# cvg/diffmvs

Hardware: AMD Instinct MI355X
Metric: depth-maps/sec (640x512, 5 src views) (higher is better)
Workload: dtype f32

## Files before the change

### diffmvs_amd/_lib.py

```python
from __future__ import annotations

import ctypes as C
import os

PKG = os.path.dirname(os.path.abspath(__file__))
HIP_LIB_PATH = os.environ.get("DMVS_LIB") or os.path.join(PKG, "libdmvs_hip.so")

ACT_NONE, ACT_RELU, ACT_SIGMOID, ACT_TANH, ACT_SILU = range(5)
IN_PLAIN, IN_UPSAMPLE2, IN_UNSHUFFLE2, IN_ZEROINSERT2 = range(4)
LAYOUT_NCHW, LAYOUT_NHWC, LAYOUT_NHWC_BF16, LAYOUT_NHWC_F16 = 0, 1, 2, 3
DTYPE_F32, DTYPE_BF16, DTYPE_F16, DTYPE_F32_PLAIN = 0, 1, 2, 3
ARITH_F32, ARITH_BF16, ARITH_SPLIT = 0, 1, 2
EW_DEPTH_TO_DISP, EW_DISP_TO_DEPTH = 0, 1

_P = C.c_void_p
_I = C.c_int32
_F = C.c_float


class Conv2dDesc(C.Structure):
    _fields_ = [
        ("in0", _P), ("in1", _P), ("mul0", _P), ("weight", _P), ("scale", _P), ("shift", _P),
        ("residual", _P), ("gru_z", _P), ("gru_h", _P), ("out", _P), ("gn_stats", _P), ("out_mul", _P),
        ("B", _I), ("c0", _I), ("c1", _I), ("Hin", _I), ("Win", _I), ("Hout", _I), ("Wout", _I),
        ("cout", _I), ("cout_pad", _I), ("kh", _I), ("kw", _I), ("stride", _I), ("pad_h", _I), ("pad_w", _I),
        ("in_mode", _I), ("act", _I), ("res_mode", _I), ("res_after_act", _I),
        ("out_layout", _I), ("out_cstride", _I), ("out_coffset", _I), ("gn_groups", _I), ("post_scale", _F),
        ("gate_cstride", _I), ("arith", _I), ("tune", _I), ("out_mul_c0", _I), ("in0_cstride", _I), ("weight_split", _P),
    ]


class Conv3dDesc(C.Structure):
    _fields_ = [
        ("in_", _P), ("weight", _P), ("scale", _P), ("shift", _P), ("residual", _P), ("out", _P),
        ("B", _I), ("cin", _I), ("cout", _I), ("cout_pad", _I),
        ("Din", _I), ("Hin", _I), ("Win", _I), ("Dout", _I), ("Hout", _I), ("Wout", _I),
        ("stride", _I), ("transposed", _I), ("act", _I), ("tune", _I),
    ]


class GetCostDesc(C.Structure):
    _fields_ = [
        ("ref", _P), ("src", _P), ("rt", _P), ("inv_depth", _P), ("confidence", _P), ("view_w", _P),
        ("disp_min", _P), ("disp_max", _P), ("out_cost", _P), ("out_samples", _P), ("worklist", _P),
        ("B", _I), ("S", _I), ("C", _I), ("G", _I), ("n", _I), ("H", _I), ("W", _I), ("vw_shift", _I),
        ("cost_cstride", _I), ("cost_coffset", _I), ("samp_cstride", _I), ("samp_coffset", _I),
        ("interval", _F), ("min_radius", _F), ("max_radius", _F), ("feat_dtype", _I), ("tune", _I),
    ]


SIGNATURES = {
    "dmvs_abi_version": [],
    "dmvs_conv2d_f32": [C.POINTER(Conv2dDesc), _P],
    "dmvs_featurenet_stem_f32": [_P, _P, _P, _P, _P, _P, _P, _P, _I, _I, _I, _I, _P],
    "dmvs_conv2d_wgrad_workspace_f32": [C.POINTER(Conv2dDesc), C.POINTER(C.c_int64)],
    "dmvs_conv2d_wgrad_f32": [C.POINTER(Conv2dDesc), _P, _P, _P, _P, C.c_int64, _P],
    "dmvs_conv3d_f32": [C.POINTER(Conv3dDesc), _P],
    "dmvs_conv3d_wgrad_workspace_f32": [C.POINTER(Conv3dDesc), C.POINTER(C.c_int64)],
    "dmvs_conv3d_wgrad_f32": [C.POINTER(Conv3dDesc), _P, _P, _P, _P, C.c_int64, _P],
    "dmvs_compose_proj_f32": [_P, _P, _I, _I, _P],
    "dmvs_warp_volume_f32": [_P, _P, _P, _P, _I, _I, _I, _I, _I, _I, _I, _P],
    "dmvs_getcost_quad_f32": [C.POINTER(GetCostDesc), _P],
    "dmvs_warp_corr_init_quad_f32": [_P, _P, _P, _P, _P, _P, _I, _I, _I, _I, _I, _I, _I, _I, _I, _I, _I, _P],
    "dmvs_warp_corr_init_bwd_f32": [_P, _P, _P, _P, _P, _P, _P, _P, _I, _I, _I, _I, _I, _I, _I, _I, _I, _I, _P],
    "dmvs_getcost_bwd_f32": [C.POINTER(GetCostDesc), _P, _P, _P, _P],
    "dmvs_view_aggregate_bwd_f32": [_P, _P, _P, _P, _P, _P, _I, _I, _I, _I, _P],
    "dmvs_view_aggregate_f32": [_P, _P, _P, _I, _I, _I, _I, _P],
    "dmvs_sigmoid_max_d_f32": [_P, _P, _I, _I, _I, _P],
    "dmvs_depth_regress_f32": [_P, _P, _P, _P, _P, _P, _I, _I, _I, _P],
    "dmvs_convex_upsample_f32": [_P, _P, _P, _P, _P, _P, _I, _I, _I, _I, _P],
    "dmvs_mask_upsample4_f32": [_P, _P, _P, _F, _P, _P, _P, _P, _P, _I, _I, _I, _I, _I, _P],
    "dmvs_groupnorm_silu_f32": [_P, _P, _P, _P, _P, _P, _P, _I, _I, _I, _I, _F, _P],
    "dmvs_groupnorm_apply_f32": [_P, _P, _P, _P, _P, _P, _P, _I, _I, _I, _I, _F, _P],
    "dmvs_delta_update_f32": [_P, _P, _P, _F, _P, _P, _P, _I, _I, _I, _I, _P],
    "dmvs_depth_convert_f32": [_P, _P, _P, _P, _I, _I, _I, _P],
    "dmvs_act_slice_f32": [_P, _P, _I, _I, _I, _I, _I, _I, _I, _I, _P],
    "dmvs_upsample_nearest_f32": [_P, _P, _I, _I, _I, _I, _P],
    "dmvs_nchw_to_nhwc_f32": [_P, _P, _I, _I, _I, _P],
    "dmvs_groupnorm_silu_bwd_workspace_f32": [_I, _I, _I, C.POINTER(C.c_int64)],
    "dmvs_groupnorm_silu_bwd_f32": [_P, _P, _P, _P, _P, _P, _P, _P, _P, _P, _P, C.c_int64, _I, _I, _I, _I, _F, _P],
    "dmvs_batchnorm_workspace_f32": [_I, _I, _I, _I, C.POINTER(C.c_int64)],
    "dmvs_batchnorm_train_fwd_f32": [_P, _P, _P, _P, _P, _P, _P, _P, _P, C.c_int64, _I, _I, _I, _I, _I, _F, _F, _I, _P],
    "dmvs_batchnorm_train_bwd_f32": [_P, _P, _P, _P, _P, _P, _P, _P, _P, _P, C.c_int64, _I, _I, _I, _I, _I, _I, _P],
    "dmvs_geo_consistency_f32": [_P, _P, _P, _P, _P, _I, _I, _F, _F, _P, _P, _I, _I, _I, _I, _I, _P],
    "dmvs_sumsq_f32": [_P, C.c_int64, _P, _P],
    "dmvs_adamw_step_f32": [_P, _P, _P, _P, C.c_int64, _F, _F, _F, _F, _F, _I, _F, _P, _F, _P],
    "dmvs_view_select_scores_f64": [_P, _P, _P, _P, _P, C.c_int64, C.c_int64, _P, _I, C.c_double, C.c_double, C.c_double, _P, _P, _P],
    "dmvs_cloud_nn_dist_f32": [_P, C.c_int64, _P, C.c_int64, _P, _P, C.c_int64, _P, C.c_double, _P, _F, _P, _P, _P],
    "dmvs_cloud_stats_f32": [_P, _P, C.c_int64, _F, _P, _I, C.c_double, _I, _P, _P],
    "dmvs_cloud_nn_index_f32": [_P, C.c_int64, _P, C.c_int64, _P, _P, C.c_int64, _P, C.c_double, _P, _F, _P, _P, _P, _P, _P],
    "dmvs_cloud_pair_moments_f64": [_P, C.c_int64, _P, _P, C.c_int64, _P, _P, _F, _P, _P, C.c_double, C.c_double, C.c_double, _I, _P, _P],
    "dmvs_cloud_crop_prism_f32": [_P, C.c_int64, _P, _P, _I, _I, C.c_double, C.c_double, _P, _P],
    "dmvs_depth_stats_f32": [_P, _P, _P, C.c_int64, C.c_int64, _P, _I, C.c_double, C.c_double, C.c_double, C.c_double, _I, _P, _P],
    "dmvs_cloud_splat_zmin_f32": [_P, C.c_int64, _P, _P, C.c_int64, _I, _I, C.c_double, C.c_double, C.c_double, _I, _I, _P, _P, _P, _P],
    "dmvs_cloud_splat_sum_f32": [_P, C.c_int64, _P, _P, C.c_int64, _I, _I, C.c_double, C.c_double, C.c_double, C.c_double, C.c_double, _I, _P, _P, _P, _P],
    "dmvs_depth_normals_f32": [_P, _P, _P, C.c_int64, _I, _I, _I, C.c_double, _I, _P, _P, _P],
}
VIEW_SELECT_MAX_IMAGES, VIEW_SELECT_MAX_LIST = 16384, 1 << 23
CLOUD_MAX_RINGS, CLOUD_MAX_KEY_BITS, CLOUD_MAX_THRESHOLDS = 1024, 62, 16
CLOUD_MOMENTS, CLOUD_MAX_POLYGON = 20, 256
DEPTH_MAX_THRESHOLDS, DEPTH_SLOTS = 8, 7
SPLAT_VIEW_CHUNK, SPLAT_VIEW_DOUBLES, SPLAT_SLOTS, SPLAT_MAX_RADIUS, SPLAT_NO_PRETEST = 8, 15, 4, 16, 0x1
NORMAL_MAX_RADIUS, NORMAL_CAM_DOUBLES, NORMAL_VIEW_CHUNK, NORMAL_SLOTS = 4, 27, 8, 4
ABI_VERSION = 4
TUNE_NO_WALK, TUNE_PIECES4, TUNE_NO_LEAN, TUNE_1X1_TILED, TUNE_NO_TALL, TUNE_TALL = 0x4, 0x8, 0x100, 0x200, 0x400, 0x800
TUNE3D_PIECES4, TUNE3D_S2_DIRECT, TUNE3D_NO_PAIR = 0x1, 0x2, 0x4
TUNE_SWEEP_GLOBAL = 0x1
TUNE_WGRAD_ACCUMULATE = 0x1000
TUNE_SPLIT_ALL = 0x20000
TUNE_STEM_EXACT = 0x40000


def tune_xcd_group(n: int) -> int:
    return (int(n) & 7) << 14


def tune3d_xcd_group(n: int) -> int:
    return (int(n) & 7) << 4
TUNE_BWD_INTERLEAVED, BWD_GATHER_INTERLEAVED = 0x1, 2


def tune_tile_wx(n: int) -> int:
    return n & 3


def tune_tile_mt(n: int) -> int:
    return (n & 7) << 4


class DmvsError(RuntimeError):
    pass


class Lib:

    def __init__(self, path: str):
        if not os.path.exists(path):
# ... 27 lines not shown
```

### diffmvs_amd/build.py

```python
from __future__ import annotations

import os
import subprocess
import sys

PKG = os.path.dirname(os.path.abspath(__file__))
ROOT = os.path.dirname(PKG)
CSRC = os.path.join(PKG, "csrc")
LIB = os.path.join(PKG, "libdmvs_hip.so")
PROBE_LIB = os.path.join(PKG, "libdmvs_probe.so")
PROBE_SOURCES = ["probe/getcost_probe.hip", "probe/random_line_gather.hip"]
SOURCES = ["conv2d_k33.hip", "conv2d_k55.hip", "conv2d_k77.hip", "conv2d_k15.hip", "conv2d.hip", "stem.hip", "conv3d.hip", "warp_quad.hip", "warp_bwd.hip", "warp_bwd_win.hip", "warp_init_bwd_win.hip", "misc.hip", "mask_upsample.hip", "optim.hip", "norm.hip", "fusion.hip", "view_select.hip", "cloud_eval.hip", "cloud_register.hip", "depth_eval.hip", "cloud_render.hip", "depth_normals.hip"]


def _deps():
    out = [os.path.join(ROOT, "include", "dmvs.h"), os.path.join(ROOT, "include", "dmvs_probe.h")]
    for base, _, files in os.walk(CSRC):
        out += [os.path.join(base, f) for f in files]
    return out


def _stale() -> bool:
    if not os.path.exists(LIB) or not os.path.exists(PROBE_LIB):
        return True
    t = min(os.path.getmtime(LIB), os.path.getmtime(PROBE_LIB))
    return any(os.path.getmtime(d) > t for d in _deps())


def build_hip(force: bool = False, save_temps: bool = False, verbose: bool = True) -> str:
    if not force and not _stale():
        return LIB
    import time
    t_start = time.time()
    hipcc = os.environ.get("HIPCC", "/opt/rocm/bin/hipcc")
    flags = ["--offload-arch=gfx950", "-O3", "-std=c++17", "-fPIC",
             "-I", os.path.join(ROOT, "include"), "-I", CSRC,
             "-munsafe-fp-atomics",
             "-Wall", "-Wno-unused-function"]
    objdir = os.path.join(ROOT, "build", "temps" if save_temps else "obj")
    os.makedirs(objdir, exist_ok=True)
    if save_temps:
        flags += ["-save-temps=obj", "-Rpass-analysis=kernel-resource-usage"]

    hdr_t = max(os.path.getmtime(d) for d in _deps() if d.endswith(".h"))

    def compile_one(src):
        obj = os.path.join(objdir, src.replace("/", "_") + ".o")
        if not force and not save_temps and os.path.exists(obj) and os.path.getmtime(obj) > max(hdr_t, os.path.getmtime(os.path.join(CSRC, src))):
            return obj
        cmd = [hipcc] + flags + ["-c", os.path.join(CSRC, src), "-o", obj]
        if verbose:
            print("[diffmvs_amd.build]", " ".join(cmd), flush=True)
        t0 = time.time()
        subprocess.run(cmd, check=True, cwd=objdir if save_temps else ROOT)
        os.utime(obj, (t0, t0))
        return obj

    from concurrent.futures import ThreadPoolExecutor
    with ThreadPoolExecutor(max_workers=min(len(SOURCES), os.cpu_count() or 4)) as pool:
        objs = list(pool.map(compile_one, SOURCES + PROBE_SOURCES))
    for lib, lobjs in ((LIB, objs[:len(SOURCES)]), (PROBE_LIB, objs[len(SOURCES):])):
        link = [hipcc, "--offload-arch=gfx950", "-shared", "-fPIC"] + lobjs + ["-o", lib]
        if verbose:
            print("[diffmvs_amd.build]", " ".join(link), flush=True)
        subprocess.run(link, check=True, cwd=ROOT)
        os.utime(lib, (t_start, t_start))
    return LIB


if __name__ == "__main__":
    build_hip(force="--force" in sys.argv, save_temps="--save-temps" in sys.argv)
    print(LIB)
```

### diffmvs_amd/engine.py

```python
from __future__ import annotations

import math
import os
from typing import Callable, Dict, List, Optional

import torch
import torch.nn.functional as F

from . import ops as K
from .ops import Ops, PackedConv, pack_conv2d, pack_conv3d

_RATIOS = [4, 2, 1]
_MULTS = [(1,), (1, 2), (1, 2, 4)]


def _bn(sd, p):
    return {k: sd[f"{p}.{k}"] for k in ("weight", "bias", "running_mean", "running_var")}


def _cw(sd, p, **kw):
    return pack_conv2d(sd[p + ".conv.weight"], sd.get(p + ".conv.bias"),
                       bn=_bn(sd, p + ".bn") if (p + ".bn.weight") in sd else None, **kw)


def pack_feature(sd, p="feature", g4=False, feat_dtype=torch.float32):
    order = (lambda w: w[K.g4_channels(w.shape[0], feat_dtype).to(w.device)].contiguous()) if g4 else (lambda w: w)
    f = {"conv0.0": _cw(sd, p + ".conv0.0", pad=1), "conv0.1": _cw(sd, p + ".conv0.1", pad=1)}
    for i in (1, 2, 3):
        f[f"conv{i}.0"] = _cw(sd, f"{p}.conv{i}.0", stride=2, pad=2)
        f[f"conv{i}.1"], f[f"conv{i}.2"] = _cw(sd, f"{p}.conv{i}.1", pad=1), _cw(sd, f"{p}.conv{i}.2", pad=1)
    f["out1"] = pack_conv2d(order(sd[p + ".out1.weight"]))
    f["inner1"] = pack_conv2d(sd[p + ".inner1.weight"], sd[p + ".inner1.bias"])
    f["out2"] = pack_conv2d(order(sd[p + ".out2.weight"]), pad=1)
    if (p + ".out3.weight") in sd:
        f["inner2"] = pack_conv2d(sd[p + ".inner2.weight"], sd[p + ".inner2.bias"])
        f["out3"] = pack_conv2d(order(sd[p + ".out3.weight"]), pad=1)
    return f


def run_feature(o: Ops, f, x, layout=K.LAYOUT_NHWC, feat_dtype=torch.float32):
    R = K.ACT_RELU
    c0 = o.featurenet_stem(f["conv0.0"], f["conv0.1"], x)
    c1 = o.conv2d(f["conv1.0"], c0, act=R)
    c1 = o.conv2d(f["conv1.2"], o.conv2d(f["conv1.1"], c1, act=R), act=R)
    c2 = o.conv2d(f["conv2.2"], o.conv2d(f["conv2.1"], o.conv2d(f["conv2.0"], c1, act=R), act=R), act=R)
    c3 = o.conv2d(f["conv3.2"], o.conv2d(f["conv3.1"], o.conv2d(f["conv3.0"], c2, act=R), act=R), act=R)
    out = {"stage1": o.conv2d(f["out1"], c3, out_layout=layout, out_dtype=feat_dtype)}
    intra = o.conv2d(f["inner1"], c2, residual=c3, res_mode=K.IN_UPSAMPLE2)
    out["stage2"] = o.conv2d(f["out2"], intra, out_layout=layout, out_dtype=feat_dtype)
    if "out3" in f:
        intra = o.conv2d(f["inner2"], c1, residual=intra, res_mode=K.IN_UPSAMPLE2)
        out["stage3"] = o.conv2d(f["out3"], intra, out_layout=layout, out_dtype=feat_dtype)
    return out


def pack_context_trunk(sd, p="context"):
    c = {"conv1": _cw(sd, p + ".conv1", pad=1)}
    for li in (1, 2, 3):
        for bi in (0, 1):
            q = f"{p}.layer{li}.{bi}"
            c[f"{li}.{bi}.conv1"] = _cw(sd, q + ".conv1", stride=(2 if bi == 0 else 1), pad=1)
            c[f"{li}.{bi}.conv2"] = _cw(sd, q + ".conv2", pad=1)
            if bi == 0:
                c[f"{li}.{bi}.down"] = _cw(sd, q + ".downsample", stride=2, pad=1)
    return c


def run_context_trunk(o: Ops, c, x):
    R = K.ACT_RELU
    x = o.conv2d(c["conv1"], x, act=R)
    taps = {}
    for li in (1, 2, 3):
        y = o.conv2d(c[f"{li}.0.conv1"], x, act=R)
        xd = o.conv2d(c[f"{li}.0.down"], x)
        x = o.conv2d(c[f"{li}.0.conv2"], y, residual=xd, act=R)
        y = o.conv2d(c[f"{li}.1.conv1"], x, act=R)
        x = o.conv2d(c[f"{li}.1.conv2"], y, residual=x, act=R)
        taps[3 - li] = x
    return taps


def pack_pvw(sd, p):
    return (pack_conv3d(sd[p + ".conv.0.conv.weight"], bn=_bn(sd, p + ".conv.0.bn")),
            pack_conv3d(sd[p + ".conv.1.weight"], sd[p + ".conv.1.bias"]))


def run_pvw(o: Ops, pk, cor):
    N, _, D, H, W = cor.shape
    x = o.conv3d(pk[1], o.conv3d(pk[0], cor, act=K.ACT_RELU))
    return o.sigmoid_max_d(x.view(N, D, H, W))


def pack_costreg(sd, p):
    reg = {}
    for i, st in ((0, 1), (1, 1), (2, 2), (3, 1), (4, 2), (5, 1)):
        reg[i] = pack_conv3d(sd[f"{p}.conv{i}.conv.weight"], bn=_bn(sd, f"{p}.conv{i}.bn"), stride=st)
    for i in (6, 7):
        reg[i] = pack_conv3d(sd[f"{p}.conv{i}.conv.weight"], bn=_bn(sd, f"{p}.conv{i}.bn"), stride=2, transposed=True)
    reg["prob"] = pack_conv3d(sd[p + ".prob.weight"])
    return reg


def run_costreg(o: Ops, reg, x):
    R = K.ACT_RELU
    c1 = o.conv3d(reg[1], o.conv3d(reg[0], x, act=R), act=R)
    c3 = o.conv3d(reg[3], o.conv3d(reg[2], c1, act=R), act=R)
    x = o.conv3d(reg[5], o.conv3d(reg[4], c3, act=R), act=R)
    x = o.conv3d(reg[6], x, act=R, residual=c3)
    x = o.conv3d(reg[7], x, act=R, residual=c1)
    return o.conv3d(reg["prob"], x)


def pack_mask(sd, p):
    return (pack_conv2d(sd[p + ".0.weight"], sd[p + ".0.bias"], pad=1), pack_conv2d(sd[p + ".2.weight"], sd[p + ".2.bias"]))


def run_mask(o: Ops, pk, context, post_scale=0.25):
    return o.conv2d(pk[1], o.conv2d(pk[0], context, act=K.ACT_RELU), post_scale=post_scale)


def mask_head_fuses(pk, up_ratio) -> bool:
    return up_ratio == 4 and pk[1].cin == 64 and pk[1].cout == 144 and pk[1].scale is None and os.environ.get("DMVS_MASK_FUSE", "1") != "0"


def pack_gru(sd, p):
    g = {}
# ... 440 lines not shown
```

### diffmvs_amd/ops.py

```python
from __future__ import annotations

import ctypes as C
import os
from dataclasses import dataclass
from typing import Optional

import torch

from . import _lib
from ._lib import (ACT_NONE, ACT_RELU, ACT_SIGMOID, ACT_SILU, ACT_TANH, ARITH_BF16, ARITH_F32, ARITH_SPLIT, DTYPE_BF16, DTYPE_F16, DTYPE_F32, IN_PLAIN,
                   IN_UNSHUFFLE2, IN_UPSAMPLE2, IN_ZEROINSERT2, LAYOUT_NCHW, LAYOUT_NHWC, LAYOUT_NHWC_BF16, LAYOUT_NHWC_F16)

CONV_ARITH = {"fp32": ARITH_F32, "bf16": ARITH_BF16, "split": ARITH_SPLIT}
FEATURE_DTYPES = {"fp32": torch.float32, "bf16": torch.bfloat16, "fp16": torch.float16}
_DTYPE_CODE = {torch.float32: DTYPE_F32, torch.bfloat16: DTYPE_BF16, torch.float16: DTYPE_F16}
_NHWC_LAYOUT = {torch.float32: LAYOUT_NHWC, torch.bfloat16: LAYOUT_NHWC_BF16, torch.float16: LAYOUT_NHWC_F16}


def _round_up(x: int, m: int) -> int:
    return (x + m - 1) // m * m


@dataclass
class PackedConv:
# ... 222 lines not shown
            if (x0.dtype != torch.float32 or x0.device != self.device or x0.stride(1) != x0.shape[2] * x0.shape[3] or
                    x0.stride(0) != in0_cstride * x0.shape[2] * x0.shape[3] or x0.stride(3) != 1 or in_mode != IN_PLAIN):
                raise _lib.DmvsError("in0_cstride: x0 must be a channel slice of a contiguous [B,in0_cstride,H,W] tensor, plain input mode")
        self._chk(out_mul)
        if gate_cstride:
            self._chk(*(() if in0_cstride else (x0,)), x1, residual, gru_h)
            for t in (mul0, gru_z):
                if t is not None and (t.dtype != torch.float32 or t.device != self.device or t.stride(1) != t.shape[2] * t.shape[3] or
                                      t.stride(0) != gate_cstride * t.shape[2] * t.shape[3] or t.stride(3) != 1):
                    raise _lib.DmvsError("gate_cstride: mul0 / gru_z must be channel slices of a contiguous [B,gate_cstride,H,W] tensor")
        else:
            self._chk(*(() if in0_cstride else (x0,)), x1, mul0, residual, gru_z, gru_h)
        if out_dtype != torch.float32:
            if out_layout != LAYOUT_NHWC or out is not None:
                raise _lib.DmvsError("16-bit outputs are channel-last feature tensors allocated by conv2d")
            out_layout = _NHWC_LAYOUT[out_dtype]
        else:
            self._chk(out)
        if gn_stats is not None and (gn_stats.dtype != torch.float64 or gn_stats.numel() < x0.shape[0] * gn_groups * 2):
            raise _lib.DmvsError("gn_stats must be float64 with B*groups*2 elements")
        B = x0.shape[0]
        if in_mode == IN_PLAIN:
            c0, Hin, Win = x0.shape[1], x0.shape[2], x0.shape[3]
        elif in_mode in (IN_UPSAMPLE2, IN_ZEROINSERT2):
            c0, Hin, Win = x0.shape[1], x0.shape[2] * 2, x0.shape[3] * 2
        else:
            c0, Hin, Win = x0.shape[1] * 4, x0.shape[2] // 2, x0.shape[3] // 2
        c1 = 0 if x1 is None else x1.shape[1]
        assert c0 + c1 == pc.cin, (c0, c1, pc.cin)
        kh, kw = pc.k
        Hout = (Hin + 2 * pc.pad[0] - kh) // pc.stride + 1
        Wout = (Win + 2 * pc.pad[1] - kw) // pc.stride + 1
        if out_cstride is None:
            out_cstride = pc.cout
        if out is None:
            shape = (B, out_cstride, Hout, Wout) if out_layout == LAYOUT_NCHW else (B, Hout, Wout, out_cstride)
            out = self.empty(*shape, dtype=out_dtype)
        arith = self.conv_arith if arith is None else arith
        wsplit = split_weights(pc) if (arith == ARITH_SPLIT and kh * kw > 1 and out_layout in (LAYOUT_NCHW, LAYOUT_NHWC)) else None
        d = _lib.Conv2dDesc(
            weight_split=_ptr(wsplit),
            in0=_ptr(x0), in1=_ptr(x1), mul0=_ptr(mul0), weight=_ptr(pc.weight), scale=_ptr(pc.scale),
            shift=_ptr(pc.shift), residual=_ptr(residual), gru_z=_ptr(gru_z), gru_h=_ptr(gru_h), out=_ptr(out),
            gn_stats=_ptr(gn_stats), gn_groups=(gn_groups if gn_stats is not None else 0), B=B, c0=c0, c1=c1, Hin=Hin, Win=Win, Hout=Hout, Wout=Wout, cout=pc.cout, cout_pad=pc.cout_pad,
            kh=kh, kw=kw, stride=pc.stride, pad_h=pc.pad[0], pad_w=pc.pad[1], in_mode=in_mode, act=act,
            res_mode=res_mode, res_after_act=int(res_after_act), out_layout=out_layout, out_cstride=out_cstride,
            out_coffset=out_coffset, post_scale=post_scale, gate_cstride=gate_cstride,
            arith=arith, tune=(self.tune["conv2d"] if tune is None else tune),
            out_mul=_ptr(out_mul), out_mul_c0=out_mul_c0, in0_cstride=in0_cstride)
        self._call("dmvs_conv2d_f32", C.byref(d), self.stream())
        if self.timers is not None and "dmvs_conv2d_f32" in self.timers:
            self.timers.setdefault("_conv2d_flops", []).append(2.0 * B * Hout * Wout * pc.cout * pc.cin * kh * kw)
            self.timers.setdefault("_conv2d_shape", []).append((B, pc.cin, pc.cout, kh, kw, pc.stride, Hout, Wout, in_mode, int(mul0 is not None)))
            nb = sum(t.numel() * t.element_size() for t in (x0, x1, mul0, residual, gru_z, gru_h, out_mul) if t is not None)
            self.timers.setdefault("_conv2d_bytes", []).append(nb + B * Hout * Wout * pc.cout * out.element_size())
        return out

    def featurenet_stem(self, pc0: PackedConv, pc1: PackedConv, x, tune=None):
        if isinstance(x, (list, tuple)):
            self._chk(*x)
            Bv, cin, H, W = x[0].shape
            y = self.empty(len(x) * Bv, 8, H, W)
            for v, xv in enumerate(x):
                self._stem_launch(pc0, pc1, xv, y[v * Bv:(v + 1) * Bv], tune)
            return y
        self._chk(x)
        N, cin, H, W = x.shape
        y = self.empty(N, 8, H, W)
        self._stem_launch(pc0, pc1, x, y, tune)
        return y

    def _stem_launch(self, pc0: PackedConv, pc1: PackedConv, x, y, tune=None):
        N, cin, H, W = x.shape
        if not (cin == 3 and pc0.cin == 3 and pc0.cout == 8 and pc1.cin == 8 and pc1.cout == 8 and pc0.k == (3, 3) and
                pc1.k == (3, 3) and pc0.stride == 1 and pc1.stride == 1 and pc0.pad == (1, 1) and pc1.pad == (1, 1) and
                pc0.cout_pad == 8 and pc1.cout_pad == 8):
            raise _lib.DmvsError("featurenet_stem: expects the 3->8->8 3x3 stem of FeatureNet")
        tune = self.tune["stem"] if tune is None else tune
        if self.conv_arith != ARITH_SPLIT:
            tune |= _lib.TUNE_STEM_EXACT
        self._call("dmvs_featurenet_stem_f32", _ptr(x), _ptr(pc0.weight), _ptr(pc0.scale), _ptr(pc0.shift), _ptr(pc1.weight),
                   _ptr(pc1.scale), _ptr(pc1.shift), _ptr(y), N, H, W, tune, self.stream())

    def conv2d_wgrad(self, pc: PackedConv, x0, grad_out, x1=None, *, mul0=None, in_mode=IN_PLAIN, want_bias=False, tune=None,
                     into_gw=None, into_gb=None):
        self._chk(x0, x1, mul0, grad_out, into_gw, into_gb)
        B = x0.shape[0]
        if in_mode == IN_PLAIN:
            c0, Hin, Win = x0.shape[1], x0.shape[2], x0.shape[3]
        elif in_mode in (IN_UPSAMPLE2, IN_ZEROINSERT2):
            c0, Hin, Win = x0.shape[1], x0.shape[2] * 2, x0.shape[3] * 2
        else:
            c0, Hin, Win = x0.shape[1] * 4, x0.shape[2] // 2, x0.shape[3] // 2
        c1 = 0 if x1 is None else x1.shape[1]
        kh, kw = pc.k
        Hout, Wout = grad_out.shape[2], grad_out.shape[3]
        acc = into_gw is not None
        if acc and (tuple(into_gw.shape) != (pc.cout, pc.cin, kh, kw) or (want_bias and (into_gb is None or tuple(into_gb.shape) != (pc.cout,)))):
            raise _lib.DmvsError("conv2d_wgrad: into_gw / into_gb do not have the gradient's shape")
        gw = into_gw if acc else self.empty(pc.cout, pc.cin, kh, kw)
        gb = (into_gb if acc else self.empty(pc.cout)) if want_bias else None
        d = _lib.Conv2dDesc(
            in0=_ptr(x0), in1=_ptr(x1), mul0=_ptr(mul0), weight=None, scale=None, shift=None, residual=None, gru_z=None,
            gru_h=None, out=None, gn_stats=None, gn_groups=0, B=B, c0=c0, c1=c1, Hin=Hin, Win=Win, Hout=Hout, Wout=Wout,
            cout=pc.cout, cout_pad=pc.cout_pad, kh=kh, kw=kw, stride=pc.stride, pad_h=pc.pad[0], pad_w=pc.pad[1],
            in_mode=in_mode, act=ACT_NONE, res_mode=IN_PLAIN, res_after_act=0, out_layout=LAYOUT_NCHW,
            out_cstride=pc.cout, out_coffset=0, post_scale=1.0, gate_cstride=0, arith=ARITH_F32,
            tune=((self.tune["conv2d"] & _lib.TUNE_PIECES4) if tune is None else tune) | (_lib.TUNE_WGRAD_ACCUMULATE if acc else 0))
        nbytes = C.c_int64(0)
        self._call("dmvs_conv2d_wgrad_workspace_f32", C.byref(d), C.byref(nbytes))
        ws = self.empty(nbytes.value // 4)
        self._call("dmvs_conv2d_wgrad_f32", C.byref(d), _ptr(grad_out), _ptr(gw), _ptr(gb), _ptr(ws), nbytes.value, self.stream())
        if self.timers is not None and "dmvs_conv2d_wgrad_f32" in self.timers:
            self.timers.setdefault("_wgrad_flops", []).append(2.0 * B * Hout * Wout * pc.cout * pc.cin * kh * kw)
        return (gw, gb) if want_bias else gw

    def conv3d(self, pc: PackedConv, x, *, act=ACT_NONE, residual=None, out=None, tune=None):
        self._chk(x, residual, out)
        B, cin, Din, Hin, Win = x.shape
        assert cin == pc.cin
        if pc.transposed:
            Dout, Hout, Wout = 2 * Din, 2 * Hin, 2 * Win
        else:
            s = pc.stride
            Dout, Hout, Wout = (Din - 1) // s + 1, (Hin - 1) // s + 1, (Win - 1) // s + 1
        if out is None:
            out = self.empty(B, pc.cout, Dout, Hout, Wout)
        d = _lib.Conv3dDesc(in_=_ptr(x), weight=_ptr(pc.weight), scale=_ptr(pc.scale), shift=_ptr(pc.shift),
                            residual=_ptr(residual), out=_ptr(out), B=B, cin=cin, cout=pc.cout, cout_pad=pc.cout_pad,
                            Din=Din, Hin=Hin, Win=Win, Dout=Dout, Hout=Hout, Wout=Wout, stride=pc.stride,
                            transposed=int(pc.transposed), act=act, tune=(self.tune["conv3d"] if tune is None else tune))
        self._call("dmvs_conv3d_f32", C.byref(d), self.stream())
        return out

    def conv3d_wgrad(self, x, grad_out, cout, stride, want_bias=False):
        self._chk(x, grad_out)
        B, cin, Din, Hin, Win = x.shape
        Dout, Hout, Wout = grad_out.shape[2:]
        gw = self.empty(cout, cin, 3, 3, 3)
        gb = self.empty(cout) if want_bias else None
        d = _lib.Conv3dDesc(in_=_ptr(x), weight=None, scale=None, shift=None, residual=None, out=None, B=B, cin=cin,
                            cout=cout, cout_pad=_pad_cout(cout), Din=Din, Hin=Hin, Win=Win, Dout=Dout, Hout=Hout, Wout=Wout,
                            stride=stride, transposed=0, act=ACT_NONE)
        nbytes = C.c_int64(0)
        self._call("dmvs_conv3d_wgrad_workspace_f32", C.byref(d), C.byref(nbytes))
        ws = self.empty(nbytes.value // 4)
        self._call("dmvs_conv3d_wgrad_f32", C.byref(d), _ptr(grad_out), _ptr(gw), _ptr(gb), _ptr(ws), nbytes.value, self.stream())
        return (gw, gb) if want_bias else gw

    def compose_proj(self, proj):
        self._chk(proj)
        B, V = proj.shape[0], proj.shape[1]
        out = self.empty(B, V - 1, 12)
        self._call("dmvs_compose_proj_f32", _ptr(proj), _ptr(out), B, V, self.stream())
        return out

    def warp_corr_init_quad(self, ref, src, rt, disp_min, disp_max, D, G=4, tune=None, plain=False):
        self._chk(rt, disp_min, disp_max)
        fdt = self._chk_feat(ref, src)
        if plain and fdt == DTYPE_F32:
            fdt = _lib.DTYPE_F32_PLAIN
        B, H, W, Cc = ref.shape
        S, _, Hs, Ws, _ = src.shape
        out = self.empty(B, S, G, D, H, W)
        self._call("dmvs_warp_corr_init_quad_f32", _ptr(ref), _ptr(src), _ptr(rt), _ptr(disp_min), _ptr(disp_max), _ptr(out),
                   B, S, Cc, G, D, H, W, Hs, Ws, fdt, self.tune["sweep"] if tune is None else tune, self.stream())
# ... 441 lines not shown
```

### include/dmvs.h

```cpp
#ifndef DMVS_H
#define DMVS_H

#include <stdint.h>

#ifdef __cplusplus
extern "C" {
#endif

#define DMVS_ABI_VERSION 4
#define DMVS_EINVAL (-22)

enum { DMVS_ACT_NONE = 0, DMVS_ACT_RELU = 1, DMVS_ACT_SIGMOID = 2, DMVS_ACT_TANH = 3, DMVS_ACT_SILU = 4 };
enum { DMVS_IN_PLAIN = 0, DMVS_IN_UPSAMPLE2 = 1 , DMVS_IN_UNSHUFFLE2 = 2 ,
       DMVS_IN_ZEROINSERT2 = 3  };
enum { DMVS_LAYOUT_NCHW = 0, DMVS_LAYOUT_NHWC = 1,
       DMVS_LAYOUT_NHWC_BF16 = 2, DMVS_LAYOUT_NHWC_F16 = 3 };
enum { DMVS_DTYPE_F32 = 0 , DMVS_DTYPE_BF16 = 1, DMVS_DTYPE_F16 = 2 ,
       DMVS_DTYPE_F32_PLAIN = 3  };

int dmvs_abi_version(void);

#define DMVS_ARITH_F32 0
#define DMVS_ARITH_BF16 1
#define DMVS_ARITH_SPLIT 2

#define DMVS_TUNE_TILE_WX(n) ((n) & 3)
#define DMVS_TUNE_NO_WALK 0x4
#define DMVS_TUNE_PIECES4 0x8
#define DMVS_TUNE_TILE_MT(n) (((n) & 7) << 4)
#define DMVS_TUNE_1X1_TILED 0x200
#define DMVS_TUNE_NO_LEAN 0x100
#define DMVS_TUNE_TALL(n) (((n) & 3) << 10)
#define DMVS_TUNE_STEM_EXACT 0x40000
#define DMVS_TUNE_SPLIT_ALL 0x20000
#define DMVS_TUNE_XCD_GROUP(n) (((n) & 7) << 14)

typedef struct dmvs_conv2d_desc {
    const float* in0;
    const float* in1;
    const float* mul0;
    const float* weight;
    const float* scale;
    const float* shift;
    const float* residual;
    const float* gru_z;
    const float* gru_h;
    float* out;
    double* gn_stats;
    const float* out_mul;
    int32_t B, c0, c1;
    int32_t Hin, Win;
    int32_t Hout, Wout;
    int32_t cout, cout_pad;
    int32_t kh, kw, stride, pad_h, pad_w;
    int32_t in_mode, act;
    int32_t res_mode;
    int32_t res_after_act;
    int32_t out_layout, out_cstride, out_coffset;
    int32_t gn_groups;
    float post_scale;
    int32_t gate_cstride;
    int32_t arith;
    int32_t tune;
    int32_t out_mul_c0;
    int32_t in0_cstride;
    const void* weight_split;
} dmvs_conv2d_desc;

int dmvs_conv2d_f32(const dmvs_conv2d_desc* d, void* stream);

int dmvs_featurenet_stem_f32(const float* x, const float* w0, const float* scale0, const float* shift0, const float* w1,
                             const float* scale1, const float* shift1, float* y, int32_t N, int32_t H, int32_t W, int32_t tune,
                             void* stream);

#define DMVS_TUNE_WGRAD_ACCUMULATE 0x1000
int dmvs_conv2d_wgrad_workspace_f32(const dmvs_conv2d_desc* d, int64_t* bytes);
int dmvs_conv2d_wgrad_f32(const dmvs_conv2d_desc* d, const float* grad_out, float* gw, float* gb, float* workspace,
                          int64_t workspace_bytes, void* stream);

typedef struct dmvs_conv3d_desc {
    const float* in;
    const float* weight;
    const float* scale;
    const float* shift;
    const float* residual;
    float* out;
    int32_t B, cin, cout, cout_pad;
    int32_t Din, Hin, Win;
    int32_t Dout, Hout, Wout;
    int32_t stride;
    int32_t transposed;
    int32_t act;
    int32_t tune;
} dmvs_conv3d_desc;
#define DMVS_TUNE3D_PIECES4 0x1
#define DMVS_TUNE3D_S2_DIRECT 0x2
#define DMVS_TUNE3D_NO_PAIR 0x4
#define DMVS_TUNE3D_XCD_GROUP(n) (((n) & 7) << 4)

int dmvs_conv3d_f32(const dmvs_conv3d_desc* d, void* stream);

int dmvs_conv3d_wgrad_workspace_f32(const dmvs_conv3d_desc* d, int64_t* bytes);
int dmvs_conv3d_wgrad_f32(const dmvs_conv3d_desc* d, const float* grad_out, float* gw, float* gb, float* workspace,
                          int64_t workspace_bytes, void* stream);

int dmvs_compose_proj_f32(const float* proj, float* out, int32_t B, int32_t V, void* stream);

#define DMVS_GETCOST_TILE 16
#define DMVS_GETCOST_MAX_WINDOW_VIEWS 16
#define DMVS_GETCOST_WORKLIST_INTS(B, H, W) \
    (4 + 66 * (B) * (((H) + DMVS_GETCOST_TILE - 1) / DMVS_GETCOST_TILE) * (((W) + DMVS_GETCOST_TILE - 1) / DMVS_GETCOST_TILE))
typedef struct dmvs_getcost_desc {
    const float* ref;
    const float* src;
    const float* rt;
    const float* inv_depth;
    const float* confidence;
    const float* view_w;
    const float* disp_min;
    const float* disp_max;
    float* out_cost;
    float* out_samples;
    int32_t* worklist;
    int32_t B, S, C, G, n, H, W;
    int32_t vw_shift;
    int32_t cost_cstride, cost_coffset, samp_cstride, samp_coffset;
    float interval, min_radius, max_radius;
    int32_t feat_dtype;
    int32_t tune;
} dmvs_getcost_desc;

#define DMVS_TUNE_SWEEP_GLOBAL 0x1
int dmvs_getcost_quad_f32(const dmvs_getcost_desc* d, void* stream);
int dmvs_warp_corr_init_quad_f32(const void* ref, const void* src, const float* rt,
                                 const float* disp_min, const float* disp_max, float* out,
                                 int32_t B, int32_t S, int32_t C, int32_t G, int32_t D,
                                 int32_t H, int32_t W, int32_t Hs, int32_t Ws, int32_t feat_dtype, int32_t tune, void* stream);

int dmvs_warp_volume_f32(const float* src, const float* rt, const float* depth, float* out,
                         int32_t B, int32_t C, int32_t D, int32_t H, int32_t W, int32_t Hs, int32_t Ws,
                         void* stream);

#define DMVS_TUNE_BWD_INTERLEAVED 0x1
#define DMVS_BWD_GATHER_INTERLEAVED 2
int dmvs_warp_corr_init_bwd_f32(const float* ref, const float* src, const float* rt,
                                const float* disp_min, const float* disp_max, const float* gcor,
                                float* gref, float* gsrc, int32_t B, int32_t S, int32_t C, int32_t G,
                                int32_t D, int32_t H, int32_t W, int32_t Hs, int32_t Ws, int32_t gather, void* stream);
int dmvs_getcost_bwd_f32(const dmvs_getcost_desc* d, const float* gcost, float* gref, float* gsrc, void* stream);
int dmvs_view_aggregate_bwd_f32(const float* cor, const float* w, const float* out, const float* gout,
                                float* gcor, float* gw, int32_t B, int32_t S, int32_t GD, int32_t HW,
                                void* stream);

int dmvs_view_aggregate_f32(const float* cor, const float* w, float* out,
                            int32_t B, int32_t S, int32_t GD, int32_t HW, void* stream);

int dmvs_sigmoid_max_d_f32(const float* x, float* out, int32_t N, int32_t D, int32_t HW, void* stream);
// ... 121 lines not shown
```

Before: 1497.

## Fuse FeatureNet stem with stride-2 5x5 conv1.0 into one streaming kernel

Adds a persistent kernel that runs both 3x3 stem convs and the 8->16 5x5 stride-2 conv1.0 in one pass over row strips. Intermediate activations stay in LDS ring buffers as split-bf16 triples, and input rows are prefetched with async global-to-LDS loads. This removes the full-resolution 8-channel c0 tensor write and read-back plus one kernel launch. It applies only under split arithmetic and is on by default via an environment switch, at the cost of heavy LDS use and extra register pressure.

```diff
diff --git a/diffmvs_amd/_lib.py b/diffmvs_amd/_lib.py
--- a/diffmvs_amd/_lib.py
+++ b/diffmvs_amd/_lib.py
@@ -53,6 +53,7 @@
     "dmvs_abi_version": [],
     "dmvs_conv2d_f32": [C.POINTER(Conv2dDesc), _P],
     "dmvs_featurenet_stem_f32": [_P, _P, _P, _P, _P, _P, _P, _P, _I, _I, _I, _I, _P],
+    "dmvs_featurenet_stem3_f32": [_P, _P, _P, _P, _P, _P, _P, _P, _P, _P, _P, _I, _I, _I, _I, _P],
     "dmvs_conv2d_wgrad_workspace_f32": [C.POINTER(Conv2dDesc), C.POINTER(C.c_int64)],
     "dmvs_conv2d_wgrad_f32": [C.POINTER(Conv2dDesc), _P, _P, _P, _P, C.c_int64, _P],
     "dmvs_conv3d_f32": [C.POINTER(Conv3dDesc), _P],
diff --git a/diffmvs_amd/build.py b/diffmvs_amd/build.py
--- a/diffmvs_amd/build.py
+++ b/diffmvs_amd/build.py
@@ -10,7 +10,7 @@
 LIB = os.path.join(PKG, "libdmvs_hip.so")
 PROBE_LIB = os.path.join(PKG, "libdmvs_probe.so")
 PROBE_SOURCES = ["probe/getcost_probe.hip", "probe/random_line_gather.hip"]
-SOURCES = ["conv2d_k33.hip", "conv2d_k55.hip", "conv2d_k77.hip", "conv2d_k15.hip", "conv2d.hip", "stem.hip", "conv3d.hip", "warp_quad.hip", "warp_bwd.hip", "warp_bwd_win.hip", "warp_init_bwd_win.hip", "misc.hip", "mask_upsample.hip", "optim.hip", "norm.hip", "fusion.hip", "view_select.hip", "cloud_eval.hip", "cloud_register.hip", "depth_eval.hip", "cloud_render.hip", "depth_normals.hip"]
+SOURCES = ["conv2d_k33.hip", "conv2d_k55.hip", "conv2d_k77.hip", "conv2d_k15.hip", "conv2d.hip", "stem.hip", "stem3.hip", "conv3d.hip", "warp_quad.hip", "warp_bwd.hip", "warp_bwd_win.hip", "warp_init_bwd_win.hip", "misc.hip", "mask_upsample.hip", "optim.hip", "norm.hip", "fusion.hip", "view_select.hip", "cloud_eval.hip", "cloud_register.hip", "depth_eval.hip", "cloud_render.hip", "depth_normals.hip"]
 
 
 def _deps():
diff --git a/diffmvs_amd/csrc/stem3.hip b/diffmvs_amd/csrc/stem3.hip
--- /dev/null
+++ b/diffmvs_amd/csrc/stem3.hip
@@ -0,0 +1,300 @@
+
+#include "dmvs_common.h"
+#include "dmvs_bf16.h"
+#include "dmvs_lds_poison.h"
+
+#include <type_traits>
+
+namespace {
+
+typedef float f32x4 __attribute__((ext_vector_type(4)));
+typedef uint32_t u32x2s __attribute__((ext_vector_type(2)));
+typedef uint32_t u32x4s __attribute__((ext_vector_type(4)));
+#define DMVS_LDS_S(p) ((__attribute__((address_space(3))) void*)(p))
+
+constexpr int UC = 32, UR = 32;
+constexpr int INW = 72;
+constexpr int INROW = 3 * INW, INGRP = 4 * INROW;
+constexpr int INSLOTS = 3;
+constexpr int INF = INSLOTS * INGRP;
+constexpr int NPIECE = INGRP / 4;
+constexpr int MW = 2 * UC + 5, CW = 2 * UC + 3;
+constexpr int MPL = 8 * MW, CPL = 8 * CW;
+constexpr int MIDF = 3 * MPL * 4, C0F = 3 * CPL * 4;
+constexpr int K0S = 9;
+constexpr int K2S = 7;
+
+__device__ __attribute__((aligned(16))) const float stem3_zero16[4] = {0.0f, 0.0f, 0.0f, 0.0f};
+
+__global__ void __launch_bounds__(DMVS_BLOCK) __attribute__((amdgpu_waves_per_eu(2, 2)))
+featurenet_stem3_kernel(const float* __restrict__ x, const float* __restrict__ w0, const float* __restrict__ scale0, const float* __restrict__ shift0,
+                        const float* __restrict__ w1, const float* __restrict__ scale1, const float* __restrict__ shift1,
+                        const float* __restrict__ w2, const float* __restrict__ scale2, const float* __restrict__ shift2, float* __restrict__ y,
+                        int N, int H, int W, int nsx, int nsy) {
+    __shared__ __attribute__((aligned(16))) float lds[INF + MIDF + C0F];
+    DMVS_LDS_POISON(lds);
+    float* const s_in = lds;
+    float* const s_mid = lds + INF;
+    float* const s_c0 = s_mid + MIDF;
+
+    const int tid = threadIdx.x, lane = tid & 63, wave = __builtin_amdgcn_readfirstlane(tid >> 6);
+    const int m = lane & 15, kq = lane >> 4;
+    const int Ho = H >> 1, Wo = W >> 1;
+    const long plane = (long)H * W, oplane = (long)Ho * Wo;
+    const int nunits = nsx * nsy * N;
+
+    float a0[K0S];
+    int koff[K0S];
+#pragma unroll
+    for (int s = 0; s < K0S; ++s) {
+        const int k = 4 * s + kq;
+        const int ci = k / 12, j = (k - ci * 12) / 3, kx = k % 3;
+        const int ky = m < 8 ? j : j - 1;
+        a0[s] = (ky >= 0 && ky <= 2) ? w0[(ci * 9 + ky * 3 + kx) * 8 + (m & 7)] : 0.0f;
+        const int koff_a = j * INROW + ci * INW + kx;
+        koff[s] = koff_a | ((koff_a + (j >= 2 ? 0 : 4 * INSLOTS * INROW)) << 16);
+    }
+    float sc0[4], sh0[4], sc1[4], sh1[4];
+#pragma unroll
+    for (int r = 0; r < 4; ++r) {
+        const int co = (4 * kq + r) & 7;
+        sc0[r] = scale0 ? scale0[co] : 1.0f;
+        sh0[r] = shift0 ? shift0[co] : 0.0f;
+        sc1[r] = scale1 ? scale1[co] : 1.0f;
+        sh1[r] = shift1 ? shift1[co] : 0.0f;
+    }
+    bf16x8 w1h[3], w1m[3], w1l[3];
+    int off1[3];
+#pragma unroll
+    for (int g = 0; g < 3; ++g) {
+        const int sl = 4 * g + kq;
+        const int j = sl / 3, kx = sl - j * 3;
+        const int ky = m < 8 ? j : j - 1;
+        float wv[8];
+#pragma unroll
+        for (int ci = 0; ci < 8; ++ci) wv[ci] = (ky >= 0 && ky <= 2) ? w1[(ci * 9 + ky * 3 + kx) * 8 + (m & 7)] : 0.0f;
+        dmvs_split3_bf16x8(wv, w1h[g], w1m[g], w1l[g]);
+        off1[g] = j | (kx << 4);
+    }
+    bf16x8 w2h[K2S], w2m[K2S], w2l[K2S];
+    int off2[K2S];
+#pragma unroll
+    for (int s = 0; s < K2S; ++s) {
+        const int sl = 4 * s + kq;
+        const int tp = min(sl, 24);
+        float wv[8];
+#pragma unroll
+        for (int ci = 0; ci < 8; ++ci) wv[ci] = sl < 25 ? w2[(ci * 25 + sl) * 16 + m] : 0.0f;
+        dmvs_split3_bf16x8(wv, w2h[s], w2m[s], w2l[s]);
+        off2[s] = (tp / 5) | ((tp % 5) << 4);
+    }
+    const float sc2 = scale2 ? scale2[m] : 1.0f, sh2 = shift2 ? shift2[m] : 0.0f;
+    const bool vec = (Wo & 3) == 0 && ((uintptr_t)y & 15) == 0;
+
+    const int p_i = tid / (NPIECE / 4), p_rem = tid - p_i * (NPIECE / 4);
+    const int p_ci = p_rem / (INW / 4), p_c = (p_rem - p_ci * (INW / 4)) * 4;
+    auto stage = [&](int unit, int kg, int slot) {
+        const int sx = unit % nsx;
+        const int uq = unit / nsx;
+        const int sy = uq % nsy, n = uq / nsy;
+        const int row = 2 * UR * sy - 5 + 4 * kg + p_i, col = 2 * UC * sx - 4 + p_c;
+        if (tid < NPIECE) {
+            const bool ok = row >= 0 && row < H && col >= 0 && col < W;
+            const float* srcp = ok ? x + ((long)n * 3 + p_ci) * plane + (long)row * W + col : stem3_zero16;
+            float* dstp = s_in + slot * INGRP + wave * 256;
+            __builtin_amdgcn_global_load_lds(srcp, DMVS_LDS_S(dstp), 16, 0, 0);
+        }
+    };
+
+    auto steps_of = [&](int unit) {
+        const int sy = (unit / nsx) % nsy;
+        return ((min(UR, Ho - UR * sy) + 1) >> 1) + 2;
+    };
+    int s_unit = blockIdx.x, s_k = 0, s_slot = 0, s_steps = s_unit < nunits ? steps_of(s_unit) : 0;
+    auto stage_next = [&]() {
+        if (s_unit < nunits) {
+            stage(s_unit, s_k, s_slot);
+            s_slot = s_slot == INSLOTS - 1 ? 0 : s_slot + 1;
+            if (++s_k == s_steps) {
+                s_unit += gridDim.x;
+                s_k = 0;
+                s_steps = s_unit < nunits ? steps_of(s_unit) : 0;
+            }
+        }
+    };
+    int islot = 0, pslot = INSLOTS - 1;
+    int unit = blockIdx.x;
+    stage_next();
+    stage_next();
+    DMVS_DMA_BARRIER();
+    for (; unit < nunits; unit += gridDim.x) {
+        const int sx = unit % nsx;
+        const int uq = unit / nsx;
+        const int sy = uq % nsy, n = uq / nsy;
+        const int X0 = 2 * UC * sx, Y0 = 2 * UR * sy, ox0 = UC * sx, oy0 = UR * sy;
+        const int nsteps = steps_of(unit);
+        for (int k = 0; k < nsteps; ++k, pslot = islot, islot = islot == INSLOTS - 1 ? 0 : islot + 1) {
+            {
+                const int sbeg = k == 0 ? MW : 0;
+                const int ng = (2 * MW - sbeg + 15) >> 4;
+                auto conv00 = [&](auto ngc, int g0) {
+                    constexpr int NG = decltype(ngc)::value;
+                    int q[NG], pm[NG];
+                    float b[NG][K0S];
+                    f32x4 acc[NG];
+#pragma unroll
+                    for (int i = 0; i < NG; ++i) {
+                        const int p = min(sbeg + (g0 + 4 * i) * 16 + m, 2 * MW - 1);
+                        q[i] = p >= MW ? 1 : 0;
+                        pm[i] = p - q[i] * MW;
+                        const int rb = q[i] ? 4 * islot : 4 * pslot + 2;
+                        const bool wrap = rb == 4 * INSLOTS - 2;
+                        const float* ip = s_in + rb * INROW + pm[i] - (wrap ? 4 * INSLOTS * INROW : 0);
+                        const int sh = wrap ? 16 : 0;
+#pragma unroll
+                        for (int s = 0; s < K0S; ++s) b[i][s] = ip[(koff[s] >> sh) & 0xffff];
+                        acc[i] = f32x4{0.0f, 0.0f, 0.0f, 0.0f};
+                    }
+#pragma unroll
+                    for (int s = 0; s < K0S; ++s)
+#pragma unroll
+                        for (int i = 0; i < NG; ++i) acc[i] = __builtin_amdgcn_mfma_f32_16x16x4f32(a0[s], b[i][s], acc[i], 0, 0, 0);
+#pragma unroll
+                    for (int i = 0; i < NG; ++i) {
+                        const int ml = 4 * k + 2 * q[i] + (kq >> 1);
+                        const int gy = Y0 - 6 + ml, gx = X0 - 3 + pm[i];
+                        const bool inside = gy >= 0 && gy < H && gx >= 0 && gx < W;
+                        if (sbeg + (g0 + 4 * i) * 16 + m < 2 * MW) {
+                            float v[8];
+#pragma unroll
+                            for (int r = 0; r < 4; ++r) {
+                                v[r] = inside ? fmaxf(fmaf(acc[i][r], sc0[r], sh0[r]), 0.0f) : 0.0f;
+                                v[4 + r] = 0.0f;
+                            }
+                            bf16x8 h8, m8, l8;
+                            dmvs_split3_bf16x8(v, h8, m8, l8);
+                            u32x2s* const d = reinterpret_cast<u32x2s*>(s_mid) + ((ml & 7) * MW + pm[i]) * 2 + (kq & 1);
+                            const u32x4s hh = __builtin_bit_cast(u32x4s, h8), mm = __builtin_bit_cast(u32x4s, m8), ll = __builtin_bit_cast(u32x4s, l8);
+                            d[0] = u32x2s{hh[0], hh[1]};
+                            d[MPL * 2] = u32x2s{mm[0], mm[1]};
+                            d[2 * MPL * 2] = u32x2s{ll[0], ll[1]};
+                        }
+                    }
+                };
+                const int cnt = (ng - wave + 3) >> 2;
+                if (cnt >= 2) conv00(std::integral_constant<int, 2>{}, wave);
+                if (cnt & 1) conv00(std::integral_constant<int, 1>{}, wave + (cnt & 2) * 4);
+            }
+            DMVS_LDS_BARRIER();
+
+            if (k >= 1) {
+                const u32x4s* const q_hi = reinterpret_cast<const u32x4s*>(s_mid);
+                for (int g = (wave + 1) & 3; g < (2 * CW + 15) / 16; g += DMVS_BLOCK / 64) {
+                    const int p = min(g * 16 + m, 2 * CW - 1);
+                    const int pr = p >= CW ? 1 : 0, pc = p - pr * CW;
+                    f32x4 acc = {0.0f, 0.0f, 0.0f, 0.0f};
+                    bf16x8 ph[3], pmid[3], pl[3];
+#pragma unroll
+                    for (int g3 = 0; g3 < 3; ++g3) {
+                        const int mr = (4 * k + 6 + 2 * pr + (off1[g3] & 15)) & 7;
+                        const int qp = mr * MW + pc + (off1[g3] >> 4);
+                        ph[g3] = __builtin_bit_cast(bf16x8, q_hi[qp]);
+                        pmid[g3] = __builtin_bit_cast(bf16x8, q_hi[MPL + qp]);
+                        pl[g3] = __builtin_bit_cast(bf16x8, q_hi[2 * MPL + qp]);
+                    }
+                    __builtin_amdgcn_sched_barrier(0);
+#pragma unroll
+                    for (int g3 = 0; g3 < 3; ++g3) {
+                        acc = dmvs_mfma_bf16(w1h[g3], pl[g3], acc);
+                        acc = dmvs_mfma_bf16(w1l[g3], ph[g3], acc);
+                        acc = dmvs_mfma_bf16(w1m[g3], pmid[g3], acc);
+                        acc = dmvs_mfma_bf16(w1h[g3], pmid[g3], acc);
+                        acc = dmvs_mfma_bf16(w1m[g3], ph[g3], acc);
+                        acc = dmvs_mfma_bf16(w1h[g3], ph[g3], acc);
+                    }
+                    const int cl = 4 * k + 2 * pr + (kq >> 1);
+                    const int gy = Y0 - 7 + cl, gx = X0 - 2 + pc;
+                    const bool inside = gy >= 0 && gy < H && gx >= 0 && gx < W;
+                    if (g * 16 + m < 2 * CW) {
+                        float v[8];
+#pragma unroll
+                        for (int r = 0; r < 4; ++r) {
+                            v[r] = inside ? fmaxf(fmaf(acc[r], sc1[r], sh1[r]), 0.0f) : 0.0f;
+                            v[4 + r] = 0.0f;
+                        }
+                        bf16x8 h8, m8, l8;
+                        dmvs_split3_bf16x8(v, h8, m8, l8);
+                        u32x2s* const d = reinterpret_cast<u32x2s*>(s_c0) + ((cl & 7) * CW + pc) * 2 + (kq & 1);
+                        const u32x4s hh = __builtin_bit_cast(u32x4s, h8), mm = __builtin_bit_cast(u32x4s, m8), ll = __builtin_bit_cast(u32x4s, l8);
+                        d[0] = u32x2s{hh[0], hh[1]};
+                        d[CPL * 2] = u32x2s{mm[0], mm[1]};
+                        d[2 * CPL * 2] = u32x2s{ll[0], ll[1]};
+                    }
+                }
+            }
+            DMVS_DMA_BARRIER();
+            stage_next();
+
+            if (k >= 2) {
+                const u32x4s* const q_hi = reinterpret_cast<const u32x4s*>(s_c0);
+                const int orow = wave >> 1, i0 = 16 * (wave & 1);
+                f32x4 acc = {0.0f, 0.0f, 0.0f, 0.0f};
+                bf16x8 ph[K2S], pmid[K2S], pl[K2S];
+                auto fetch = [&](int s) {
+                    const int cr = (4 * k + 5 + 2 * orow + (off2[s] & 15)) & 7;
+                    const int qp = cr * CW + 2 * (i0 + m) + (off2[s] >> 4);
+                    ph[s] = __builtin_bit_cast(bf16x8, q_hi[qp]);
+                    pmid[s] = __builtin_bit_cast(bf16x8, q_hi[CPL + qp]);
+                    pl[s] = __builtin_bit_cast(bf16x8, q_hi[2 * CPL + qp]);
+                };
+                fetch(0);
+                fetch(1);
+#pragma unroll
+                for (int s = 0; s < K2S; ++s) {
+                    if (s + 2 < K2S) fetch(s + 2);
+                    __builtin_amdgcn_sched_barrier(0);
+                    acc = dmvs_mfma_bf16(pl[s], w2h[s], acc);
+                    acc = dmvs_mfma_bf16(ph[s], w2l[s], acc);
+                    acc = dmvs_mfma_bf16(pmid[s], w2m[s], acc);
+                    acc = dmvs_mfma_bf16(pmid[s], w2h[s], acc);
+                    acc = dmvs_mfma_bf16(ph[s], w2m[s], acc);
+                    acc = dmvs_mfma_bf16(ph[s], w2h[s], acc);
+                    __builtin_amdgcn_sched_barrier(0);
+                }
+                const int oy = oy0 + 2 * (k - 2) + orow, ox = ox0 + i0 + 4 * kq;
+                if (oy < Ho && ox < Wo) {
+                    f32x4 v;
+#pragma unroll
+                    for (int r = 0; r < 4; ++r) v[r] = fmaxf(fmaf(acc[r], sc2, sh2), 0.0f);
+                    float* dst = y + ((long)n * 16 + m) * oplane + (long)oy * Wo + ox;
+                    if (vec) {
+                        *reinterpret_cast<f32x4*>(dst) = v;
+                    } else {
+#pragma unroll
+                        for (int r = 0; r < 4; ++r)
+                            if (ox + r < Wo) dst[r] = v[r];
+                    }
+                }
+            }
+        }
+    }
+}
+
+}
+
+extern "C" int dmvs_featurenet_stem3_f32(const float* x, const float* w0, const float* scale0, const float* shift0, const float* w1,
+                                         const float* scale1, const float* shift1, const float* w2, const float* scale2, const float* shift2,
+                                         float* y, int32_t N, int32_t H, int32_t W, int32_t tune, void* stream) {
+    (void)tune;
+    if (!x || !w0 || !w1 || !w2 || !y || N <= 0 || H <= 0 || W <= 0) return DMVS_EINVAL;
+    if ((long)3 * H * W >= (1L << 31)) return DMVS_EINVAL;
+    if ((H & 1) || (W & 3) || ((uintptr_t)x & 15)) return DMVS_EINVAL;
+    const int nsx = (W / 2 + UC - 1) / UC, nsy = (H / 2 + UR - 1) / UR;
+    const long nunits = (long)nsx * nsy * N;
+    if (nunits >= (1L << 31)) return DMVS_EINVAL;
+    static const int resident = dmvs_resident_workgroups(reinterpret_cast<const void*>(featurenet_stem3_kernel));
+    const unsigned grid = (unsigned)(nunits < resident ? nunits : resident);
+    hipLaunchKernelGGL(featurenet_stem3_kernel, dim3(grid), dim3(DMVS_BLOCK), 0, (hipStream_t)stream, x, w0, scale0, shift0, w1, scale1, shift1, w2,
+                       scale2, shift2, y, N, H, W, nsx, nsy);
+    return dmvs_launch_status();
+}
diff --git a/diffmvs_amd/engine.py b/diffmvs_amd/engine.py
--- a/diffmvs_amd/engine.py
+++ b/diffmvs_amd/engine.py
@@ -38,10 +38,21 @@
     return f
 
 
+STEM_FUSE_DEFAULT = "1"
+
+
+def stem3_applies(o: Ops, x):
+    return (o.conv_arith == K.ARITH_SPLIT and os.environ.get("DMVS_STEM_FUSE", STEM_FUSE_DEFAULT) != "0" and
+            o.featurenet_stem3_supported(x))
+
+
 def run_feature(o: Ops, f, x, layout=K.LAYOUT_NHWC, feat_dtype=torch.float32):
     R = K.ACT_RELU
-    c0 = o.featurenet_stem(f["conv0.0"], f["conv0.1"], x)
-    c1 = o.conv2d(f["conv1.0"], c0, act=R)
+    if stem3_applies(o, x):
+        c1 = o.featurenet_stem3(f["conv0.0"], f["conv0.1"], f["conv1.0"], x)
+    else:
+        c0 = o.featurenet_stem(f["conv0.0"], f["conv0.1"], x)
+        c1 = o.conv2d(f["conv1.0"], c0, act=R)
     c1 = o.conv2d(f["conv1.2"], o.conv2d(f["conv1.1"], c1, act=R), act=R)
     c2 = o.conv2d(f["conv2.2"], o.conv2d(f["conv2.1"], o.conv2d(f["conv2.0"], c1, act=R), act=R), act=R)
     c3 = o.conv2d(f["conv3.2"], o.conv2d(f["conv3.1"], o.conv2d(f["conv3.0"], c2, act=R), act=R), act=R)
diff --git a/diffmvs_amd/ops.py b/diffmvs_amd/ops.py
--- a/diffmvs_amd/ops.py
+++ b/diffmvs_amd/ops.py
@@ -328,6 +328,30 @@
         self._call("dmvs_featurenet_stem_f32", _ptr(x), _ptr(pc0.weight), _ptr(pc0.scale), _ptr(pc0.shift), _ptr(pc1.weight),
                    _ptr(pc1.scale), _ptr(pc1.shift), _ptr(y), N, H, W, tune, self.stream())
 
+    @staticmethod
+    def featurenet_stem3_supported(x):
+        xs = x if isinstance(x, (list, tuple)) else [x]
+        H, W = xs[0].shape[2], xs[0].shape[3]
+        return H % 2 == 0 and W % 4 == 0 and 3 * H * W < 2 ** 31 and all(t.data_ptr() % 16 == 0 for t in xs)
+
+    def featurenet_stem3(self, pc0: PackedConv, pc1: PackedConv, pc2: PackedConv, x, tune=None):
+        xs = x if isinstance(x, (list, tuple)) else [x]
+        self._chk(*xs)
+        Bv, cin, H, W = xs[0].shape
+        if not (cin == 3 and pc0.cin == 3 and pc0.cout == 8 and pc1.cin == 8 and pc1.cout == 8 and pc0.k == (3, 3) and
+                pc1.k == (3, 3) and pc0.stride == 1 and pc1.stride == 1 and pc0.pad == (1, 1) and pc1.pad == (1, 1) and
+                pc0.cout_pad == 8 and pc1.cout_pad == 8 and pc2.cin == 8 and pc2.cout == 16 and pc2.cout_pad == 16 and pc2.k == (5, 5) and
+                pc2.stride == 2 and pc2.pad == (2, 2)):
+            raise _lib.DmvsError("featurenet_stem3: expects the 3->8->8 3x3 stem of FeatureNet and its 8->16 5x5 stride-2 conv1.0")
+        if not self.featurenet_stem3_supported(xs) or any(t.shape != xs[0].shape for t in xs):
+            raise _lib.DmvsError(f"featurenet_stem3: needs even H, W % 4 == 0 and 16-byte aligned views of one shape, got {tuple(xs[0].shape)}")
+        y = self.empty(len(xs) * Bv, 16, H // 2, W // 2)
+        for v, xv in enumerate(xs):
+            self._call("dmvs_featurenet_stem3_f32", _ptr(xv), _ptr(pc0.weight), _ptr(pc0.scale), _ptr(pc0.shift), _ptr(pc1.weight),
+                       _ptr(pc1.scale), _ptr(pc1.shift), _ptr(pc2.weight), _ptr(pc2.scale), _ptr(pc2.shift), _ptr(y[v * Bv:(v + 1) * Bv]),
+                       Bv, H, W, 0 if tune is None else tune, self.stream())
+        return y
+
     def conv2d_wgrad(self, pc: PackedConv, x0, grad_out, x1=None, *, mul0=None, in_mode=IN_PLAIN, want_bias=False, tune=None,
                      into_gw=None, into_gb=None):
         self._chk(x0, x1, mul0, grad_out, into_gw, into_gb)
diff --git a/include/dmvs.h b/include/dmvs.h
--- a/include/dmvs.h
+++ b/include/dmvs.h
@@ -73,6 +73,10 @@
                              const float* scale1, const float* shift1, float* y, int32_t N, int32_t H, int32_t W, int32_t tune,
                              void* stream);
 
+int dmvs_featurenet_stem3_f32(const float* x, const float* w0, const float* scale0, const float* shift0, const float* w1,
+                              const float* scale1, const float* shift1, const float* w2, const float* scale2, const float* shift2,
+                              float* y, int32_t N, int32_t H, int32_t W, int32_t tune, void* stream);
+
 #define DMVS_TUNE_WGRAD_ACCUMULATE 0x1000
 int dmvs_conv2d_wgrad_workspace_f32(const dmvs_conv2d_desc* d, int64_t* bytes);
 int dmvs_conv2d_wgrad_f32(const dmvs_conv2d_desc* d, const float* grad_out, float* gw, float* gb, float* workspace,
```

Result: faster. 1520, median of 6 (+1.5%).
